# Gabrielcb/DaliID

Measured on AMD Instinct MI355X. Metric: images/sec (train step), higher is better.
Workload: dtype bf16; 1 GPU; configs[1]: ResNet-50 ReID bf16 256x128, PK batch 16x16=256 per GPU, center+proxy heads, Adam, EMA; global_batch=256, per_gpu_batch=256, parallelism=dp1

## Files before the change

daliid_amd/csrc/conv.hip:

```cpp
#include "gemm_tile.h"
#include "kernels.h"
#include <cstdlib>
#include <type_traits>
#include <vector>
#include <string>
#include <cstdio>

namespace dali {

__device__ __forceinline__ void decode_pixel(const GatherGeom& g, int p, int& n, int& ho, int& wo) {
    if (g.lhw >= 0 && g.lw >= 0) {
        n = p >> g.lhw;
        const int rem = p & ((1 << g.lhw) - 1);
        ho = rem >> g.lw;
        wo = rem & ((1 << g.lw) - 1);
    } else {
        const int hw = g.Hout * g.Wout;
        n = p / hw;
        const int rem = p - n * hw;
        ho = rem / g.Wout;
        wo = rem - ho * g.Wout;
    }
}

// ... 1370 lines not shown
    const int bn = n0 + c16 * 8;
    const bool b_ok = bn < a.Ntot;
    const int tap = b_ok ? bn / g.Ck : 0;
    const int ci = bn - tap * g.Ck;
    const int r = tap / g.S, s = tap - r * g.S;
    const int p_begin = wk.p_begin, p_end = wk.p_end, ksteps = wk.ksteps;

    auto issue = [&](int kt, int stage) {
        uint16_t* sa = smem + stage * 2 * TILE;
        uint16_t* sb = sa + TILE;
#pragma unroll
        for (int i = 0; i < 2; ++i) {
            const int blk = wave + 4 * i;
            const int p = p_begin + kt * 32 + 4 * blk + r_in;
            uint32_t oa = DMA_OOB, ob = DMA_OOB;
            if (p < p_end) {
                if (a_ok) oa = (uint32_t)(p * a.Cm + am) * 2u;
                if (b_ok) {
                    int n, ho, wo;
                    decode_pixel(g, p, n, ho, wo);
                    const int hi = ho * g.stride - g.pad + r, wi = wo * g.stride - g.pad + s;
                    if ((unsigned)hi < (unsigned)g.Hin && (unsigned)wi < (unsigned)g.Win)
                        ob = (uint32_t)((int)((long long)n * g.img_pitch) + hi * g.row_pitch + wi * g.pix_pitch + ci) * 2u;
                }
            }
            __builtin_amdgcn_raw_ptr_buffer_load_lds(rs.y, (lds_void_ptr)(sa + blk * 512), 16, oa, 0, 0, 0);
            __builtin_amdgcn_raw_ptr_buffer_load_lds(rs.x, (lds_void_ptr)(sb + blk * 512), 16, ob, 0, 0, 0);
        }
    };

    f32x4_t acc[4][4];
#pragma unroll
    for (int i = 0; i < 4; ++i)
#pragma unroll
        for (int j = 0; j < 4; ++j) acc[i][j] = f32x4_t{0.f, 0.f, 0.f, 0.f};
    const bool do_cs = COLSUM && tn == 0 && wn == 0;
    f32x4_t cs[4];
#pragma unroll
    for (int i = 0; i < 4; ++i) cs[i] = f32x4_t{0.f, 0.f, 0.f, 0.f};
    typedef short ones_vec_t __attribute__((ext_vector_type(8)));
    const bf16x8_t ones = __builtin_bit_cast(bf16x8_t, ones_vec_t{0x3F80, 0x3F80, 0x3F80, 0x3F80, 0x3F80, 0x3F80, 0x3F80, 0x3F80});

    if (ksteps > 0) {
        issue(0, 0);
        if (ksteps > 1) issue(1, 1);
        if (ksteps > 1) dma_wait<4>(); else dma_wait<0>();
        __builtin_amdgcn_s_barrier();
        conv_stamp(a, 1);
        int st_cur = 0, st_nxt2 = 2;
        for (int kt = 0; kt < ksteps; ++kt) {
            if (kt + 2 < ksteps) issue(kt + 2, st_nxt2);
            const uint16_t* sa = smem + st_cur * 2 * TILE;
            const uint16_t* sb = sa + TILE;
            bf16x8_t fa[4];
            wgrad_tr_kstep(sa, wm * 4, sb, wn * 4, lane, acc, fa);
            if constexpr (COLSUM) if (do_cs) {
#pragma unroll
                for (int i = 0; i < 4; ++i) cs[i] = __builtin_amdgcn_mfma_f32_16x16x32_bf16(fa[i], ones, cs[i], 0, 0, 0);
            }
            if (kt + 2 < ksteps) dma_wait<4>(); else dma_wait<0>();
            __builtin_amdgcn_s_barrier();
            st_cur = (st_cur == 2) ? 0 : st_cur + 1;
            st_nxt2 = (st_nxt2 == 2) ? 0 : st_nxt2 + 1;
        }
    }
    conv_stamp(a, 2);
    float* slab = a.partial + (size_t)ks * a.Cm * a.Ntot;
    store_slab_tiles<4, 4>(slab, acc, m0 + wm * 64, n0 + wn * 64, a.Cm, a.Ntot, lane);
    if constexpr (COLSUM) if (do_cs && (lane & 15) == 0) {
#pragma unroll
        for (int i = 0; i < 4; ++i)
#pragma unroll
            for (int rr = 0; rr < 4; ++rr) {
                const int m = m0 + wm * 64 + i * 16 + (lane >> 4) * 4 + rr;
                if (m < a.Cm) a.colsum[(size_t)ks * a.Cm + m] = cs[i][rr];
            }
    }
    conv_stamp_stores(a);
}

__device__ __forceinline__ int halo_swz(int row) { return ((row >> 1) & 1) | (((row >> 3) & 1) << 1); }
constexpr int W3_A_ELEMS = 32 * 128, W3_B_ELEMS = 16 * 512, W3_STAGE = W3_A_ELEMS + W3_B_ELEMS;

template <int NSTAGE>
__global__ __launch_bounds__(512) void igemm_wgrad3x3_kernel(WGradArgs a, int tiles_m, int tiles_n) {
    extern __shared__ __attribute__((aligned(16))) uint16_t smem[];
    const int tid = threadIdx.x, lane = tid & 63;
    const int wave = __builtin_amdgcn_readfirstlane(tid >> 6);
    const int wm = wave >> 2, wn = wave & 3;
    WGradWork wk;
    if (!wk.map_xcd(a, tiles_m, tiles_n)) return;
    const int ks = wk.ks, m0 = wk.tm * 128, ci0 = wk.tn * 64;
    conv_stamp(a, 0);
    const bool m_active = m0 + wm * 64 < a.Cm;
    const GatherGeom g = a.g;
    const int W = g.Wout, H = g.Hout, Cin = g.Ck, lw = g.lw, lhw = g.lhw;
    const int RW = 32 >> lw, HC = W + 2, HP = (RW + 2) * HC;
    const WGradRsrc rs = wgrad_rsrc(a);

    const int r_in = lane >> 4, ps = lane & 15;
    const int c16 = ((((ps >> 1) ^ wg_swz(4 * wave + r_in)) << 1) | (ps & 1));
    const int am = m0 + c16 * 8;
    const bool a_ok = am < a.Cm;
    int hb_hr[2], hb_off[2];
    bool hb_ok[2];
#pragma unroll
    for (int i = 0; i < 2; ++i) {
        const int hp = 8 * (wave + 8 * i) + (lane >> 3);
        const int lc = (lane & 7) ^ (halo_swz(hp) << 1);
        const int hr = hp / HC, hc = hp - hr * HC;
        hb_hr[i] = hr;
        hb_ok[i] = hp < HP && (unsigned)(hc - 1) < (unsigned)W && ci0 + lc * 8 < Cin;
        hb_off[i] = ((hc - 1) * Cin + ci0 + lc * 8) * 2;
    }
    const int p_begin = wk.p_begin, p_end = wk.p_end, ksteps = wk.ksteps;

    auto issue = [&](int kt, int stage) {
        uint16_t* sa = smem + stage * W3_STAGE;
        uint16_t* sb = sa + W3_A_ELEMS;
        const int p0 = p_begin + kt * 32;
        const int p = p0 + 4 * wave + r_in;
        const uint32_t oa = (p < p_end && a_ok) ? (uint32_t)(p * a.Cm + am) * 2u : DMA_OOB;
        __builtin_amdgcn_raw_ptr_buffer_load_lds(rs.y, (lds_void_ptr)(sa + wave * 512), 16, oa, 0, 0, 0);
        const int n = p0 >> lhw, h_base = (p0 & ((1 << lhw) - 1)) >> lw;
        const int row_bytes = W * Cin * 2;
        const int img_base = (int)((long long)n * g.img_pitch * 2);
#pragma unroll
        for (int i = 0; i < 2; ++i) {
            const int h = h_base - 1 + hb_hr[i];
            const bool ok = hb_ok[i] && (unsigned)h < (unsigned)H && p0 < p_end;
            const uint32_t ob = ok ? (uint32_t)(img_base + h * row_bytes + hb_off[i]) : DMA_OOB;
            __builtin_amdgcn_raw_ptr_buffer_load_lds(rs.x, (lds_void_ptr)(sb + (wave + 8 * i) * 512), 16, ob, 0, 0, 0);
        }
    };

    f32x4_t acc[9][4];
#pragma unroll
    for (int t = 0; t < 9; ++t)
#pragma unroll
        for (int i = 0; i < 4; ++i) acc[t][i] = f32x4_t{0.f, 0.f, 0.f, 0.f};
    const int gq = lane >> 4, q = (lane & 15) >> 2, pp = lane & 3;
    const int hrow_base = ((8 * gq) >> lw) * HC + ((8 * gq) & (W - 1)) + q;
    int boff0[9], boff1[9];
#pragma unroll
    for (int r = 0; r < 3; ++r)
#pragma unroll
        for (int s2 = 0; s2 < 3; ++s2) {
            const int row0 = hrow_base + r * HC + s2, row1 = row0 + 4;
            boff0[r * 3 + s2] = row0 * 64 + ((wn ^ halo_swz(row0)) << 4) + 4 * pp;
            boff1[r * 3 + s2] = row1 * 64 + ((wn ^ halo_swz(row1)) << 4) + 4 * pp;
        }
    auto load_b = [&](const uint16_t* sb, int t) -> TrPair { return TrPair{ds_read_tr_raw(sb + boff0[t]), ds_read_tr_raw(sb + boff1[t])}; };

    constexpr int AHEAD = NSTAGE - 1;
    auto wait_inflight = [&](int n) {
        if (n <= 0) dma_wait<0>();
        else if (n == 1) dma_wait<3>();
        else if (n == 2) dma_wait<6>();
        else if (n == 3) dma_wait<9>();
        else dma_wait<12>();
    };
    static_assert(AHEAD >= 1 && AHEAD <= 5, "ring depth");
    if (ksteps > 0) {
        int issued = 0;
        for (; issued < AHEAD && issued < ksteps; ++issued) issue(issued, issued);
        wait_inflight(issued - 1 > 4 ? 4 : issued - 1);
        __builtin_amdgcn_s_barrier();
        conv_stamp(a, 1);
        int st_cur = 0, st_fill = AHEAD % NSTAGE;
        for (int kt = 0; kt < ksteps; ++kt) {
            if (kt + AHEAD < ksteps) issue(kt + AHEAD, st_fill);
            const uint16_t* sa = smem + st_cur * W3_STAGE;
            const uint16_t* sb = sa + W3_A_ELEMS;
            if (m_active) {
            TrPair ra[4], rb[9];
#pragma unroll
            for (int i = 0; i < 4; ++i) ra[i] = tr_frag_raw(sa, wm * 4 + i, lane);
#pragma unroll
            for (int t = 0; t < 9; ++t) rb[t] = load_b(sb, t);
            tr_settle<18>(ra[0], ra[1], ra[2], ra[3]);
            tr_settle<10>(rb[0], rb[1], rb[2], rb[3]);
            bf16x8_t fa[4];
#pragma unroll
            for (int i = 0; i < 4; ++i) fa[i] = tr_join(ra[i]);
#pragma unroll
            for (int t = 0; t < 4; ++t) {
                const bf16x8_t fb = tr_join(rb[t]);
#pragma unroll
                for (int i = 0; i < 4; ++i) acc[t][i] = __builtin_amdgcn_mfma_f32_16x16x32_bf16(fa[i], fb, acc[t][i], 0, 0, 0);
            }
            __builtin_amdgcn_sched_barrier(0);
            tr_settle<0>(rb[4], rb[5], rb[6], rb[7]);
            tr_settle_all(rb[8]);
#pragma unroll
            for (int t = 4; t < 9; ++t) {
                const bf16x8_t fb = tr_join(rb[t]);
#pragma unroll
                for (int i = 0; i < 4; ++i) acc[t][i] = __builtin_amdgcn_mfma_f32_16x16x32_bf16(fa[i], fb, acc[t][i], 0, 0, 0);
            }
            }
            const int left = ksteps - 1 - kt;
            const int keep = (left < AHEAD ? left : AHEAD) - 1;
            wait_inflight(keep > 4 ? 4 : keep);
            __builtin_amdgcn_s_barrier();
            st_cur = (st_cur == NSTAGE - 1) ? 0 : st_cur + 1;
            st_fill = (st_fill == NSTAGE - 1) ? 0 : st_fill + 1;
        }
    }
    conv_stamp(a, 2);
    float* slab = a.partial + (size_t)ks * a.Cm * a.Ntot;
    if (m_active) {
        float* row = slab + (size_t)(m0 + wm * 64 + (lane >> 4) * 4) * a.Ntot + ci0 + wn * 16 + (lane & 15);
#pragma unroll
        for (int i = 0; i < 4; ++i)
#pragma unroll
            for (int rr = 0; rr < 4; ++rr) {
                float* p = row + (size_t)(i * 16 + rr) * a.Ntot;
#pragma unroll
                for (int t = 0; t < 9; ++t) p[t * Cin] = acc[t][i][rr];
            }
    }
    conv_stamp_stores(a);
}

template <int WM, int WN, int NSTAGE, bool COLSUM = false>
__global__ __launch_bounds__(WM * WN * 64, 4) void igemm_wgrad_wg_kernel(WGradArgs a, int tiles_m, int tiles_n) {
    constexpr int TM = 64 * WM, TN = 64 * WN, NW = WM * WN;
    using Gather = WGradGather<TM / 128, (TM + TN) / 128, NW>;
    constexpr int IMG = Gather::IMG, NIMG_A = Gather::NIMG_A, STAGE = Gather::STAGE, NDMA = Gather::NDMA;
    constexpr int AHEAD = NSTAGE - 1;
    static_assert(TM % 128 == 0 && TN % 128 == 0, "unsupported wave grid");
    extern __shared__ __attribute__((aligned(16))) uint16_t smem[];
    const int tid = threadIdx.x, lane = tid & 63;
    const int wave = __builtin_amdgcn_readfirstlane(tid >> 6);
    const int wm = wave / WN, wn = wave % WN;
    WGradWork wk;
    if (!wk.map_xcd(a, tiles_m, tiles_n)) return;
    const int m0 = wk.tm * TM, n0 = wk.tn * TN, ksteps = wk.ksteps;
    const Gather gather(a, wave, m0, n0, wk.p_begin, wk.p_end, lane);

    const bool do_cs = COLSUM && wn == 0;
    int cs_turn = wk.tn;
    f32x4_t cs = f32x4_t{0.f, 0.f, 0.f, 0.f};
    typedef unsigned sel_vec_t __attribute__((ext_vector_type(4)));
    const int cs_col = (lane & 15) >> 2;
    f32x4_t acc[4][4];
// ... 351 lines not shown

int gemm_profile_begin(hipStream_t st, int cls, double flops, const char* what) {
    if (!g_prof || g_prof->used >= g_prof->cap) return -1;
    const size_t i = g_prof->used++;
    g_prof->cls[i] = cls; g_prof->flops[i] = flops; g_prof->desc[i] = what;
    (void)hipEventRecord(g_prof->ev[2 * i], st);
    return (int)i;
}
void gemm_profile_end(hipStream_t st, int slot) {
    if (slot >= 0 && g_prof) (void)hipEventRecord(g_prof->ev[2 * slot + 1], st);
}

enum GemmGrid {
    GRID_XCD,
    GRID_CLASSES,
    GRID_CUS,
    GRID_HALO,
    GRID_SPLITS,
    GRID_SPLITS8,
};
struct GemmKernel {
    const void* fn;
    int block;
    int lds;
    int tm, tn;
    GemmGrid grid;
    int plan_wgs = 0;
    int f1_rb = 0;
    mutable DeviceOnce once{};
};
template <class F> static const void* kfn(F* f) { return reinterpret_cast<const void*>(f); }
constexpr int ring_lds(int tm, int tn, int k_tile, int stages) { return (tm + tn) * k_tile * 2 * stages; }
constexpr int REG128_LDS = GemmCfg<128, 128, 1, 1, 1>::LDS_BYTES, REG64_LDS = GemmCfg<64, 256, 1, 1, 1>::LDS_BYTES;
constexpr int DMA128_LDS = REG128_LDS / 2 * 3, DMA64_LDS = REG64_LDS / 2 * 3;
constexpr int HALO64_LDS = (3 * 64 * 64 + HALO64_PX * 64) * 2;

static const GemmKernel
    CONV128_BN{kfn(&igemm_conv_kernel<128, 128, true>), 256, REG128_LDS, 128, 128, GRID_XCD},
    CONV128{kfn(&igemm_conv_kernel<128, 128, false>), 256, REG128_LDS, 128, 128, GRID_XCD},
    DMA128{kfn(&igemm_conv_dma_kernel<128, 128, 3>), 256, DMA128_LDS, 128, 128, GRID_XCD},
    DMA128_LIN{kfn(&igemm_conv_dma_kernel<128, 128, 3, Epi::LIN>), 256, DMA128_LDS, 128, 128, GRID_XCD},
    DMA128_FUSED{kfn(&igemm_conv_dma_kernel<128, 128, 3, Epi::FUSED>), 256, DMA128_LDS, 128, 128, GRID_XCD},
    DMA128_CLS{kfn(&igemm_conv_dma_kernel<128, 128, 3, Epi::PARITY>), 256, DMA128_LDS, 128, 128, GRID_CLASSES},
    DMA128_SRC2{kfn(&igemm_conv_dma_kernel<128, 128, 3, Epi::CONV, true>), 256, DMA128_LDS, 128, 128, GRID_XCD},
    CONV64_BN{kfn(&igemm_conv_kernel<64, 256, true>), 256, REG64_LDS, 64, 256, GRID_XCD},
    CONV64{kfn(&igemm_conv_kernel<64, 256, false>), 256, REG64_LDS, 64, 256, GRID_XCD},
    DMA64{kfn(&igemm_conv_dma_kernel<64, 256, 3>), 256, DMA64_LDS, 64, 256, GRID_XCD},
    DMA64_LEAN{kfn(&igemm_conv_dma_kernel<64, 256, 3, Epi::FUSED_LEAN>), 256, DMA64_LDS, 64, 256, GRID_XCD},
    DMA64_SRC2{kfn(&igemm_conv_dma_kernel<64, 256, 3, Epi::CONV, true>), 256, DMA64_LDS, 64, 256, GRID_XCD},
    K64S64{kfn(&igemm_conv_k64s_kernel<1, 4, 4, 2>), 512, ring_lds(64, 256, 64, 2), 64, 256, GRID_XCD},
    HALO64{kfn(&igemm_conv_halo64_kernel<3>), 512, HALO64_LDS, 64, 256, GRID_HALO},
    HALO64_LEAN{kfn(&igemm_conv_halo64_kernel<3, Epi::FUSED_LEAN>), 512, HALO64_LDS, 64, 256, GRID_HALO},
    WG128{kfn(&igemm_conv_wg_kernel<2, 4, 3>), 512, ring_lds(128, 256, 32, 3), 128, 256, GRID_XCD},
    WG128_LIN{kfn(&igemm_conv_wg_kernel<2, 4, 3, Epi::LIN>), 512, ring_lds(128, 256, 32, 3), 128, 256, GRID_XCD},
    WG128_FUSED{kfn(&igemm_conv_wg_kernel<2, 4, 3, Epi::FUSED>), 512, ring_lds(128, 256, 32, 3), 128, 256, GRID_XCD},
    WG128_CLS{kfn(&igemm_conv_wg_kernel<2, 4, 3, Epi::PARITY>), 512, ring_lds(128, 256, 32, 3), 128, 256, GRID_CLASSES},
    WG256{kfn(&igemm_conv_wg_kernel<4, 4, 4>), 1024, ring_lds(256, 256, 32, 4), 256, 256, GRID_XCD},
    K64S{kfn(&igemm_conv_k64s_kernel<2, 4, 8, 3>), 1024, ring_lds(128, 256, 64, 3), 128, 256, GRID_XCD},
    K64S_LIN{kfn(&igemm_conv_k64s_kernel<2, 4, 8, 3, 4, 4, Epi::LIN>), 1024, ring_lds(128, 256, 64, 3), 128, 256, GRID_XCD},
    K64S_LEAN{kfn(&igemm_conv_k64s_kernel<2, 4, 8, 3, 4, 4, Epi::FUSED_LEAN>), 1024, ring_lds(128, 256, 64, 3), 128, 256, GRID_XCD},
    K64S_SRC2{kfn(&igemm_conv_k64s_kernel<2, 4, 8, 3, 4, 4, Epi::CONV, true>), 1024, ring_lds(128, 256, 64, 3), 128, 256, GRID_XCD},
    K64{kfn(&igemm_conv_k64_kernel<4, 4, 2>), 1024, ring_lds(256, 256, 64, 2), 256, 256, GRID_XCD},
    K64_LIN{kfn(&igemm_conv_k64_kernel<4, 4, 2, 4, 4, Epi::LIN>), 1024, ring_lds(256, 256, 64, 2), 256, 256, GRID_XCD},
    K64_FUSED{kfn(&igemm_conv_k64_kernel<4, 4, 2, 4, 4, Epi::FUSED>), 1024, ring_lds(256, 256, 64, 2), 256, 256, GRID_XCD},
    K64_CLS{kfn(&igemm_conv_k64_kernel<4, 4, 2, 4, 4, Epi::PARITY>), 1024, ring_lds(256, 256, 64, 2), 256, 256, GRID_CLASSES},
    K64_SRC2{kfn(&igemm_conv_k64_kernel<4, 4, 2, 4, 4, Epi::CONV, true>), 1024, ring_lds(256, 256, 64, 2), 256, 256, GRID_XCD},
    K64_FUSED_SRC2{kfn(&igemm_conv_k64_kernel<4, 4, 2, 4, 4, Epi::FUSED, true>), 1024, ring_lds(256, 256, 64, 2), 256, 256, GRID_XCD},
    K64_320{kfn(&igemm_conv_k64_kernel<4, 4, 2, 4, 5, Epi::LIN>), 1024, ring_lds(256, 320, 64, 2), 256, 320, GRID_XCD};

template <int RB, bool RES, bool OM, bool BITS, bool SRC2 = false>
static GemmKernel f1_kernel() {
    return {kfn(&fused1x1_persist_kernel<3, RB, RES, OM, BITS, SRC2>), (F1_NC + F1_NP + F1_NR) * 64, f1_lds_bytes(3, RB, RB == 2 ? 128 : F1_KMAX),
            F1_TM, F1_TN, GRID_CUS, 0, RB};
}
static const GemmKernel F1[2][2][2][2] = {
    {{{f1_kernel<2, false, false, false, true>(), f1_kernel<2, false, false, true>()}, {f1_kernel<2, false, true, false>(), f1_kernel<2, false, true, true>()}},
     {{f1_kernel<2, true, false, false>(), f1_kernel<2, true, false, true>()}, {f1_kernel<2, true, true, false>(), f1_kernel<2, true, true, true>()}}},
    {{{f1_kernel<1, false, false, false, true>(), f1_kernel<1, false, false, true>()}, {f1_kernel<1, false, true, false>(), f1_kernel<1, false, true, true>()}},
     {{f1_kernel<1, true, false, false>(), f1_kernel<1, true, false, true>()}, {f1_kernel<1, true, true, false>(), f1_kernel<1, true, true, true>()}}}};

static const GemmKernel
    WG_BN{kfn(&igemm_wgrad_kernel<true>), 256, 0, 128, 128, GRID_SPLITS},
    WG_PLAIN{kfn(&igemm_wgrad_kernel<false>), 256, 0, 128, 128, GRID_SPLITS},
    WG_3X3{kfn(&igemm_wgrad3x3_kernel<3>), 512, 3 * W3_STAGE * 2, 128, 9 * 64, GRID_SPLITS8, 256};
static const GemmKernel WG_DMA[2] = {
    {kfn(&igemm_wgrad_dma_kernel<false>), 256, 0, 128, 128, GRID_SPLITS8},
    {kfn(&igemm_wgrad_dma_kernel<true>), 256, 0, 128, 128, GRID_SPLITS8}};
static const GemmKernel WG_WG[2] = {
    {kfn(&igemm_wgrad_wg_kernel<2, 4, 3>), 512, ring_lds(128, 256, 32, 3), 128, 256, GRID_SPLITS8, 512},
    {kfn(&igemm_wgrad_wg_kernel<2, 4, 3, true>), 512, ring_lds(128, 256, 32, 3), 128, 256, GRID_SPLITS8, 512}};
static const GemmKernel WG_P[2][2] = {
    {{kfn(&igemm_wgrad_p_kernel<2, 4, 4, 4, 8, 6>), 1024, ring_lds(128, 256, 32, 6), 128, 256, GRID_SPLITS8, 256},
     {kfn(&igemm_wgrad_p_kernel<2, 4, 4, 4, 8, 6, true>), 1024, ring_lds(128, 256, 32, 6), 128, 256, GRID_SPLITS8, 256}},
    {{kfn(&igemm_wgrad_p_kernel<1, 4, 8, 4, 4, 6>), 512, ring_lds(128, 256, 32, 6), 128, 256, GRID_SPLITS8, 256},
     {kfn(&igemm_wgrad_p_kernel<1, 4, 8, 4, 4, 6, true>), 512, ring_lds(128, 256, 32, 6), 128, 256, GRID_SPLITS8, 256}}};

struct GemmChoice {
    const GemmKernel* k = nullptr;
    int tiles_m = 0, tiles_n = 0, lds = 0, class_grid = 0;
    unsigned grid = 0;
    int rc = DALI_OK, why_arg = 0;
    const char* why = nullptr;
    GemmChoice() = default;
    GemmChoice(int rc_, const char* why_, int why_arg_ = 0) : rc(rc_), why_arg(why_arg_), why(why_) {}
    int refuse() const { set_error(why, why_arg); return rc; }
};
static GemmChoice gemm_place(const GemmKernel& k, int rows, int cols, int mult, int Ck) {
    GemmChoice c;
    c.k = &k;
    c.tiles_m = (rows + k.tm - 1) / k.tm;
    c.tiles_n = (cols + k.tn - 1) / k.tn;
    c.lds = k.f1_rb ? f1_lds_bytes(3, k.f1_rb, Ck) : k.lds;
    switch (k.grid) {
        case GRID_XCD: c.grid = xcd_tile_grid(c.tiles_m, c.tiles_n); break;
        case GRID_CLASSES: c.class_grid = xcd_tile_grid(c.tiles_m, c.tiles_n); c.grid = mult * c.class_grid; break;
        case GRID_CUS: c.grid = mult; break;
        case GRID_HALO: c.grid = c.tiles_n; break;
        case GRID_SPLITS: c.grid = c.tiles_m * c.tiles_n * mult; break;
        case GRID_SPLITS8: c.grid = (c.tiles_m * c.tiles_n * mult + 7) / 8 * 8; break;
    }
    return c;
}
template <class Args>
static int gemm_launch(hipStream_t st, const GemmChoice& c, Args& args) {
    const GemmKernel& k = *c.k;
    DeviceOnce::Guard once(k.once);
    if (k.lds > 64 * 1024 && once.first()) {
        DALI_HIP(hipFuncSetAttribute(k.fn, hipFuncAttributeMaxDynamicSharedMemorySize, k.lds));
        once.done();
    }
    int tiles_m = c.tiles_m, tiles_n = c.tiles_n;
    void* tile_args[] = {&args, &tiles_m, &tiles_n};
    void* halo_args[] = {&args, &tiles_n};
    (void)hipLaunchKernel(k.fn, dim3(c.grid), dim3(k.block), k.grid == GRID_HALO ? halo_args : tile_args, c.lds, st);
    DALI_LAUNCH_CHECK();
    return DALI_OK;
}

static unsigned long long* g_conv_stamps = nullptr;

static bool dma_addressable(long long bytes) { return bytes < 0x7ff00000ll; }
static bool gather_dma_ok(const GatherGeom& g, int P, long long other_bytes) {
    return dma_addressable(g.img_pitch * 2 * ((P + g.Hout * g.Wout - 1) / (g.Hout * g.Wout))) && dma_addressable(other_bytes);
}
static bool conv_dma_ok(const IGemmArgs& a) { return !a.in_scale && gather_dma_ok(a.g, a.P, (long long)a.Cm * a.g.R * a.g.S * a.g.Ck * 2); }
static bool plain_rows(const GatherGeom& g) {
    return g.R == 1 && g.S == 1 && g.stride == 1 && g.pad == 0 && g.pix_pitch == g.Ck && g.row_pitch == g.Win * g.Ck &&
           g.img_pitch == (long long)g.Hin * g.Win * g.Ck && g.Hin == g.Hout && g.Win == g.Wout;
}
static bool halo64_ok(const IGemmArgs& a) {
    const GatherGeom& g = a.g;
    return a.Cm == 64 && g.Ck == 64 && g.R == 3 && g.S == 3 && g.stride == 1 && g.pad == 1 && !g.sub && (g.Wout == 16 || g.Wout == 32) &&
           ilog2_exact(g.Hout * g.Wout) >= 8 && g.Hin == g.Hout && g.Win == g.Wout && g.pix_pitch == 64 && g.row_pitch == g.Win * 64 &&
           g.img_pitch == (long long)g.Hin * g.Win * 64 && a.P % 256 == 0;
}

static int f1_cu_count() {
    static int n_cus = 0;
    if (!n_cus) {
        int dev = 0, v = 0;
        if (hipGetDevice(&dev) != hipSuccess || hipDeviceGetAttribute(&v, hipDeviceAttributeMultiprocessorCount, dev) != hipSuccess) { set_error("conv: device query failed"); return -1; }
        n_cus = v > 8 ? v & ~7 : 8;
    }
    return n_cus;
}
static bool f1_fills(int Cm, int P, int n_cus) {
    const int tiles_m = Cm / F1_TM, tiles_n = (P + F1_TN - 1) / F1_TN;
// ... 65 lines not shown
    if (k64 && cfg == CONV_256x256) return use(a.X2 ? K64_SRC2 : lin ? K64_LIN : K64);
    if (k64 && cfg == CONV_128x256) return use(a.X2 ? K64S_SRC2 : lin ? K64S_LIN : K64S);
    if (narrow_k64 && !lin && halo64_ok(a)) return use(HALO64);
    if (narrow_k64) return use(K64S64);
    if (narrow) return use(in_bn ? CONV64_BN : !dma_ok ? CONV64 : a.X2 ? DMA64_SRC2 : DMA64);
    if (dma_ok && cfg == CONV_256x256) return use(WG256);
    if (dma_ok && cfg == CONV_128x256) return use(lin ? WG128_LIN : WG128);
    return use(in_bn ? CONV128_BN : !dma_ok ? CONV128 : a.X2 ? DMA128_SRC2 : lin ? DMA128_LIN : DMA128);
}

static int launch_igemm_conv_one(hipStream_t st, const IGemmArgs& a) {
    IGemmArgs args = a;
    args.g.lw = ilog2_exact(a.g.Wout);
    args.g.lhw = ilog2_exact(a.g.Hout * a.g.Wout);
    const GemmChoice c = conv_choose(args, f1_cu_count());
    if (c.rc == DALI_ERR_LIMIT) return c.refuse();
    const int K = a.g.nr * a.g.ns * a.g.Ck;
    char what[160] = "";
    if (g_prof)
        snprintf(what, sizeof what, "%s,Cm=%d,K=%d,P=%d,taps=%d,stride=%d,sub=%d,fused=%d,stats=%d,res=%d,mask=%d,lin=%d", a.g.mode ? "dgrad" : "fwd", a.Cm, K, a.P,
                 a.g.R * a.g.S, a.g.stride, a.g.sub, a.out_scale ? 1 : 0, a.stats ? 1 : 0, a.Res ? 1 : 0, (a.res_mask || a.out_mask) ? 1 : 0,
                 (a.bias || a.row_scale || a.act) ? 1 : 0);
    ProfScope prof_scope(st, 0, a.g.sub == 2 ? 2.0 * a.Cm * (double)a.P * a.g.R * a.g.S * a.g.Ck : 2.0 * a.Cm * (double)a.P * K, what);
    if (!c.k) return c.refuse();
    const int stat_tiles = a.stats ? igemm_conv_stat_tiles(a.Cm, a.P, K, a.in_scale != nullptr) : c.tiles_n;
    if (stat_tiles != c.tiles_n) {
        set_error("conv: the statistics slab has %d pixel tiles, the chosen kernel %d", stat_tiles, c.tiles_n);
        return DALI_ERR_UNSUPPORTED;
    }
    if (c.k->grid == GRID_CLASSES) args.g.class_grid = c.class_grid;
    return gemm_launch(st, c, args);
}

int launch_igemm_conv(hipStream_t st, const IGemmArgs& a) {
    IGemmArgs args = a;
    args.stamps = g_conv_stamps;
    GatherGeom& g = args.g;
    g.sub = 0; g.oph = g.opw = 0; g.Hfull = g.Hout; g.Wfull = g.Wout;
    g.r0 = 0; g.rstep = 1; g.nr = g.R; g.s0 = 0; g.sstep = 1; g.ns = g.S;
    if (g.mode == 1 && g.stride == 2 && conv_dma_ok(args) && !a.stats && (g.Hout % 2) == 0 && (g.Wout % 2) == 0 &&
        ilog2_exact(g.Wout / 2) >= 0 && ilog2_exact((g.Hout / 2) * (g.Wout / 2)) >= 0) {
        int nr[2], ns[2];
        for (int ph = 0; ph < 2; ++ph) {
            const int r0 = (ph + g.pad) & 1, s0 = (ph + g.pad) & 1;
            nr[ph] = r0 < g.R ? (g.R - r0 + 1) / 2 : 0;
            ns[ph] = s0 < g.S ? (g.S - s0 + 1) / 2 : 0;
        }
        const bool all_have = nr[0] && nr[1] && ns[0] && ns[1];
        if (all_have && a.Cm > 64 && (a.Cm & 7) == 0) {
            IGemmArgs s = args;
            s.g.sub = 2; s.g.oph = s.g.opw = 0; s.g.Hfull = g.Hout; s.g.Wfull = g.Wout;
            s.g.Hout = g.Hout / 2; s.g.Wout = g.Wout / 2; s.P = a.P / 4;
            s.g.r0 = s.g.s0 = 0; s.g.rstep = s.g.sstep = 2;
            s.g.nr = nr[0] > nr[1] ? nr[0] : nr[1]; s.g.ns = ns[0] > ns[1] ? ns[0] : ns[1];
            return launch_igemm_conv_one(st, s);
        }
        if (all_have || (a.Res != nullptr && a.Res == a.O)) {
            for (int ph = 0; ph < 2; ++ph)
                for (int pw = 0; pw < 2; ++pw) {
                    if (nr[ph] * ns[pw] == 0) continue;
                    IGemmArgs s = args;
                    s.g.sub = 1; s.g.oph = ph; s.g.opw = pw; s.g.Hfull = g.Hout; s.g.Wfull = g.Wout;
                    s.g.Hout = g.Hout / 2; s.g.Wout = g.Wout / 2; s.P = a.P / 4;
                    s.g.r0 = (ph + g.pad) & 1; s.g.rstep = 2; s.g.nr = nr[ph];
                    s.g.s0 = (pw + g.pad) & 1; s.g.sstep = 2; s.g.ns = ns[pw];
                    const int rc = launch_igemm_conv_one(st, s);
                    if (rc) return rc;
                }
            return DALI_OK;
        }
    }
    return launch_igemm_conv_one(st, args);
}

static bool wgrad_spec(int Cm, int Ntot) { return ((Cm + 127) / 128) * ((Ntot + 255) / 256) <= 100; }
int wgrad_pick_cfg(int Cm, int Ntot, int taps, int P, int halo_w) {
    if (taps == 9 && (halo_w == 8 || halo_w == 16 || halo_w == 32) && Cm % 64 == 0 && (Ntot / 9) % 64 == 0 && P % 32 == 0) return 3;
    if (taps == 7 && Ntot == 224 && P >= 16384) return 2;
    return (taps == 1 && Ntot >= 256 && P >= 16384) ? 2 : 0;
}
static const GemmKernel& wgrad_kernel(int cfg, int Cm, int Ntot, bool in_bn, bool dma_ok, bool colsum, bool flat) {
    if (in_bn) return WG_BN;
    if (!dma_ok) return WG_PLAIN;
    if (cfg == 3) return WG_3X3;
    if (cfg == 2) return wgrad_spec(Cm, Ntot) ? WG_P[flat][colsum] : WG_WG[colsum];
    return WG_DMA[colsum];
}
static bool wgrad_colsum_ok(int cfg, bool in_bn, bool dma_ok) { return cfg != 3 && !in_bn && dma_ok; }
static int colsum_rows_of(const GemmKernel& k, int Ntot, int splits) { return k.tn == 128 ? splits : splits * ((Ntot + k.tn - 1) / k.tn); }

void wgrad_plan(int Cm, int Ntot, int P, int target_blocks, int* splits, int* pix_per_split, size_t* ws_bytes, int taps, int halo_w) {
    const GemmKernel& k = wgrad_kernel(wgrad_pick_cfg(Cm, Ntot, taps, P, halo_w), Cm, Ntot, false, true, false, true);
    if (k.plan_wgs) target_blocks = k.plan_wgs;
    const int tiles = ((Cm + k.tm - 1) / k.tm) * ((Ntot + k.tn - 1) / k.tn);
    int sp = (target_blocks + tiles - 1) / tiles;
    const int max_sp = (P + 255) / 256;
    if (sp > max_sp) sp = max_sp;
    if (sp < 1) sp = 1;
    {
        int best = sp;
        double best_cost = (double)((tiles * sp + target_blocks - 1) / target_blocks) / sp;
        for (int c = sp - 1; c >= 1 && c >= sp / 2; --c) {
            const double cost = (double)((tiles * c + target_blocks - 1) / target_blocks) / c;
            if (cost <= best_cost + 1e-12) { best = c; best_cost = cost; }
        }
        sp = best;
    }
    int pps = ((P + sp - 1) / sp + 31) & ~31;
    sp = (P + pps - 1) / pps;
    *splits = sp; *pix_per_split = pps;
    *ws_bytes = (size_t)sp * Cm * Ntot * sizeof(float);
}

static GemmChoice wgrad_choose(const WGradArgs& a) {
    const GatherGeom& g = a.g;
    const bool dma_ok = gather_dma_ok(g, a.P, (long long)a.P * a.Cm * 2);
    const bool halo = g.R == 3 && g.S == 3 && g.stride == 1 && g.pad == 1 && g.mode == 0 && g.lw >= 0 && g.lhw >= 7 && g.Hin == g.Hout && g.Win == g.Wout &&
                      g.pix_pitch == g.Ck && g.row_pitch == g.Win * g.Ck;
    const int cfg = wgrad_pick_cfg(a.Cm, a.Ntot, g.R * g.S, a.P, halo ? g.Wout : 0);
    if (a.colsum && !wgrad_colsum_ok(cfg, a.in_scale != nullptr, dma_ok))
        return GemmChoice(DALI_ERR_INVALID, "wgrad: column sums ride on the 128 x 128 and 128 x 256 LDS-DMA kernels only (wgrad_colsum_supported)");
    return gemm_place(wgrad_kernel(cfg, a.Cm, a.Ntot, a.in_scale != nullptr, dma_ok, a.colsum != nullptr, plain_rows(g)), a.Cm, a.Ntot, a.splits, g.Ck);
}

int launch_igemm_wgrad(hipStream_t st, const WGradArgs& a, float* out, int accumulate, float* colsum_out, int colsum_rows) {
    WGradArgs args = a;
    args.stamps = g_conv_stamps;
    args.g.lw = ilog2_exact(a.g.Wout);
    args.g.lhw = ilog2_exact(a.g.Hout * a.g.Wout);
    const GemmChoice c = wgrad_choose(args);
    {
    char what[160] = "";
    if (g_prof)
        snprintf(what, sizeof what, "wgrad,Cm=%d,K=%d,P=%d,taps=%d,stride=%d,sub=0,fused=%d,stats=0,res=0,mask=0,lin=%d", a.Cm, a.Ntot, a.P, a.g.R * a.g.S, a.g.stride,
                 a.in_scale ? 1 : 0, a.colsum ? 1 : 0);
    ProfScope prof_scope(st, 1, 2.0 * a.Cm * (double)a.Ntot * a.P, what);
    if (!c.k) return c.refuse();
    if (a.colsum && colsum_out && colsum_rows != colsum_rows_of(*c.k, a.Ntot, a.splits)) {
        set_error("wgrad: %d column-sum rows passed, the chosen kernel leaves %d", colsum_rows, colsum_rows_of(*c.k, a.Ntot, a.splits));
        return DALI_ERR_UNSUPPORTED;
    }
    if (int rc = gemm_launch(st, c, args)) return rc;
    }
    if (!out) return DALI_OK;
    return launch_splitk_reduce2(st, a.partial, out, (size_t)a.Cm * a.Ntot, a.splits, accumulate, (a.colsum && colsum_out) ? a.colsum : nullptr, colsum_out,
                                 (size_t)a.Cm, colsum_rows);
}

int wgrad_colsum_rows(int Cm, int Ntot, int taps, int P, int splits) {
    return colsum_rows_of(wgrad_kernel(wgrad_pick_cfg(Cm, Ntot, taps, P, 0), Cm, Ntot, false, true, true, true), Ntot, splits);
}
bool wgrad_colsum_supported(int Cm, int Ntot, int taps, int P) {
    return wgrad_colsum_ok(wgrad_pick_cfg(Cm, Ntot, taps, P, 0), false, dma_addressable((long long)P * Cm * 2) && dma_addressable((long long)P * Ntot * 2));
}

int launch_splitk_reduce(hipStream_t st, const float* partial, float* out, size_t elems, int splits, int accumulate) {
    return launch_splitk_reduce2(st, partial, out, elems, splits, accumulate, nullptr, nullptr, 0, 0);
}
int launch_splitk_reduce2(hipStream_t st, const float* partial, float* out, size_t elems, int splits, int accumulate,
                          const float* partial2, float* out2, size_t elems2, int splits2) {
    const size_t chunks = (elems + 3) / 4;
    const unsigned rblocks = (unsigned)((chunks + 63) / 64);
    const int W = splits >= 32 ? 16 : (splits >= 2 ? 4 : 1);
    const bool second = partial2 && out2 && elems2 > 0;
    if (second && ((elems & 3) || (elems2 & 3))) {
        if (int rc = launch_splitk_reduce2(st, partial, out, elems, splits, accumulate, nullptr, nullptr, 0, 0)) return rc;
        return launch_splitk_reduce2(st, partial2, out2, elems2, splits2, 0, nullptr, nullptr, 0, 0);
    }
    if (elems & 3) {
        hipLaunchKernelGGL(splitk_reduce_odd_kernel, dim3((unsigned)((elems + 255) / 256)), dim3(256), 0, st, partial, out, elems, splits, accumulate, W);
        DALI_LAUNCH_CHECK();
        return DALI_OK;
    }
    ReduceJob2 j2{nullptr, nullptr, 0, 0, 0xffffffffu};
    unsigned grid = rblocks;
    if (second) { j2 = ReduceJob2{partial2, out2, elems2, splits2, rblocks}; grid += (unsigned)((elems2 / 4 + 63) / 64); }
    switch (W) {
        case 1: hipLaunchKernelGGL(splitk_reduce_kernel<1>, dim3(grid), dim3(64), 0, st, partial, out, elems, splits, accumulate, j2); break;
        case 4: hipLaunchKernelGGL(splitk_reduce_kernel<4>, dim3(grid), dim3(256), 0, st, partial, out, elems, splits, accumulate, j2); break;
        default: hipLaunchKernelGGL(splitk_reduce_kernel<16>, dim3(grid), dim3(1024), 0, st, partial, out, elems, splits, accumulate, j2); break;
    }
    DALI_LAUNCH_CHECK();
    return DALI_OK;
}

}

extern "C" int dali_debug_set_conv_stamps(void* dev_ptr) { g_conv_stamps = static_cast<unsigned long long*>(dev_ptr); return DALI_OK; }
extern "C" int dali_debug_wgrad_splits(int Cm, int Ntot, int P, int taps, int halo_w) {
    int sp = 0, pps = 0; size_t wsb = 0;
    wgrad_plan(Cm, Ntot, P, 512, &sp, &pps, &wsb, taps, halo_w);
    return sp;
}
extern "C" int dali_debug_splitk_reduce(void* stream, const float* partial, float* out, long long elems, int splits, int accumulate) {
    return launch_splitk_reduce(static_cast<hipStream_t>(stream), partial, out, (size_t)elems, splits, accumulate);
}

extern "C" int dali_gemm_profile_begin(dali_ctx* ctx, int max_launches) {
    DALI_REQUIRE(ctx && max_launches > 0, "dali_gemm_profile_begin: bad argument");
    DALI_REQUIRE(!g_prof, "dali_gemm_profile_begin: a profile is already open");
    GemmProfiler* p = new GemmProfiler();
    p->cap = (size_t)max_launches;
    p->ev.resize(2 * p->cap); p->cls.resize(p->cap); p->flops.resize(p->cap); p->desc.resize(p->cap);
    for (auto& e : p->ev) DALI_HIP(hipEventCreate(&e));
    g_prof = p;
    return DALI_OK;
}

extern "C" int dali_gemm_profile_end(dali_ctx* ctx, double* total_ms, double* total_flops, long long* launches) {
    DALI_REQUIRE(ctx && total_ms && total_flops && launches, "dali_gemm_profile_end: null argument");
    DALI_REQUIRE(g_prof, "dali_gemm_profile_end: no open profile");
    GemmProfiler* p = g_prof;
    g_prof = nullptr;
    for (int c = 0; c < 2; ++c) { total_ms[c] = 0; total_flops[c] = 0; launches[c] = 0; }
    int rc = DALI_OK;
    const char* dump_path = getenv("DALI_GEMM_PROFILE_DUMP");
    FILE* dump = dump_path ? fopen(dump_path, "a") : nullptr;
    for (size_t i = 0; i < p->used; ++i) {
        float ms = 0.f;
        if (hipEventSynchronize(p->ev[2 * i + 1]) != hipSuccess || hipEventElapsedTime(&ms, p->ev[2 * i], p->ev[2 * i + 1]) != hipSuccess) {
            set_error("gemm_profile_end: event query failed"); rc = DALI_ERR_HIP; break;
        }
        total_ms[p->cls[i]] += ms; total_flops[p->cls[i]] += p->flops[i]; launches[p->cls[i]] += 1;
        if (dump) fprintf(dump, "%zu,%s,us=%.2f,gflop=%.3f\n", i, p->desc[i].c_str(), ms * 1e3, p->flops[i] * 1e-9);
    }
    if (dump) fclose(dump);
    for (auto& e : p->ev) (void)hipEventDestroy(e);
    delete p;
    return rc;
}

static int fill_geom(GatherGeom& g, int n_img, int Hin, int Win, int Ck, int Hout, int Wout, int R, int S, int stride, int pad, int mode) {
    g.Hout = Hout; g.Wout = Wout; g.Hin = Hin; g.Win = Win; g.Ck = Ck; g.R = R; g.S = S; g.stride = stride; g.pad = pad;
    g.mode = mode;
    g.pix_pitch = Ck; g.row_pitch = Win * Ck; g.img_pitch = (long long)Hin * Win * Ck;
    g.lw = g.lhw = -1;
    (void)n_img;
    return 0;
}

extern "C" int dali_conv2d_fwd(dali_ctx* ctx, void* stream, const uint16_t* x, const uint16_t* w, uint16_t* y,
                               int n, int h, int wd, int cin, int cout, int r, int s, int stride, int pad,
                               const float* in_scale, const float* in_shift, int in_relu, float* stats) {
    DALI_REQUIRE(ctx && x && w && y, "dali_conv2d_fwd: null argument");
    DALI_REQUIRE(cin % 32 == 0 && cout % 4 == 0, "dali_conv2d_fwd: cin must be a multiple of 32 and cout of 4 (cin=%d cout=%d)", cin, cout);
    DALI_REQUIRE(stride == 1 || stride == 2, "dali_conv2d_fwd: stride %d unsupported", stride);
    DALI_REQUIRE((in_scale == nullptr) == (in_shift == nullptr), "dali_conv2d_fwd: in_scale/in_shift must come together");
    const int ho = (h + 2 * pad - r) / stride + 1, wo = (wd + 2 * pad - s) / stride + 1;
    IGemmArgs a{};
    a.W = w; a.X = x; a.O = y; a.Res = nullptr; a.in_scale = in_scale; a.in_shift = in_shift; a.stats = stats;
    a.Cm = cout; a.P = n * ho * wo; a.in_relu = in_relu;
    fill_geom(a.g, n, h, wd, cin, ho, wo, r, s, stride, pad, 0);
    return launch_igemm_conv((hipStream_t)stream, a);
}

extern "C" int dali_conv2d_bn_act(dali_ctx* ctx, void* stream, const uint16_t* x, const uint16_t* w, uint16_t* y, int n, int h, int wd, int cin, int cout,
                                  int r, int s, int stride, int pad, const float* out_scale, const float* out_shift, int out_relu) {
    DALI_REQUIRE(ctx && x && w && y && out_scale && out_shift, "dali_conv2d_bn_act: null argument");
    DALI_REQUIRE(cin % 32 == 0 && cout % 8 == 0, "dali_conv2d_bn_act: cin must be a multiple of 32 and cout of 8 (cin=%d cout=%d)", cin, cout);
    DALI_REQUIRE(stride == 1 || stride == 2, "dali_conv2d_bn_act: stride %d unsupported", stride);
    const int ho = (h + 2 * pad - r) / stride + 1, wo = (wd + 2 * pad - s) / stride + 1;
    IGemmArgs a{};
    a.W = w; a.X = x; a.O = y;
    a.out_scale = out_scale; a.out_shift = out_shift; a.out_relu = out_relu;
    a.Cm = cout; a.P = n * ho * wo;
    fill_geom(a.g, n, h, wd, cin, ho, wo, r, s, stride, pad, 0);
    return launch_igemm_conv((hipStream_t)stream, a);
}

static int halo_width(int r, int s, int stride, int pad, int ho, int wo) {
    return (r == 3 && s == 3 && stride == 1 && pad == 1 && ilog2_exact(wo) >= 0 && ilog2_exact(ho * wo) >= 0 && ho * wo >= 128) ? wo : 0;
}
extern "C" int dali_conv2d_stat_tiles(int cout, int cin, int r, int s, int stride, int pad, int n, int ho, int wo, int fused_operand) {
    (void)stride; (void)pad;
    return igemm_conv_stat_tiles(cout, n * ho * wo, r * s * cin, fused_operand != 0);
// ... 145 lines not shown
```

include/daliid_debug.h:

```cpp
#ifndef DALIID_DEBUG_H
#define DALIID_DEBUG_H

#ifdef __cplusplus
extern "C" {
#endif

int dali_debug_reload_env(void);

int dali_debug_set_conv_stamps(void* dev_ptr);

int dali_debug_wgrad_splits(int Cm, int Ntot, int P, int taps, int halo_w);

int dali_debug_splitk_reduce(void* stream, const float* partial, float* out, long long elems, int splits, int accumulate);

struct dali_resnet;
int dali_debug_resnet_backward_block(struct dali_resnet* net, void* stream, const float* d_emb, int block);

#ifdef __cplusplus
}
#endif
#endif
```

Baseline: 17810 images/s.

## Split k-steps across wave halves in 3x3 wgrad kernel when Cm is 64

Adds a KPAIR variant of the 3x3 weight-gradient kernel for layers with Cm<=64. In the existing kernel the upper-M waves have no work for these layers. In the new variant the two wave rows each process alternate k-steps from a deeper six-stage ring. Their accumulators are then summed through LDS at the end. This aims to use the otherwise idle waves in layer1's 64-channel 3x3 convs, at the cost of twice the LDS footprint and an extra LDS reduction.

```diff
diff --git a/daliid_amd/csrc/conv.hip b/daliid_amd/csrc/conv.hip
--- a/daliid_amd/csrc/conv.hip
+++ b/daliid_amd/csrc/conv.hip
@@ -1476,7 +1476,7 @@
 __device__ __forceinline__ int halo_swz(int row) { return ((row >> 1) & 1) | (((row >> 3) & 1) << 1); }
 constexpr int W3_A_ELEMS = 32 * 128, W3_B_ELEMS = 16 * 512, W3_STAGE = W3_A_ELEMS + W3_B_ELEMS;
 
-template <int NSTAGE>
+template <int NSTAGE, bool KPAIR = false>
 __global__ __launch_bounds__(512) void igemm_wgrad3x3_kernel(WGradArgs a, int tiles_m, int tiles_n) {
     extern __shared__ __attribute__((aligned(16))) uint16_t smem[];
     const int tid = threadIdx.x, lane = tid & 63;
@@ -1555,7 +1555,77 @@
         else dma_wait<12>();
     };
     static_assert(AHEAD >= 1 && AHEAD <= 5, "ring depth");
-    if (ksteps > 0) {
+    if constexpr (KPAIR) {
+        constexpr int NSLOT = NSTAGE / 2, AHEAD2 = NSLOT - 1;
+        static_assert(NSTAGE % 2 == 0 && AHEAD2 >= 1 && AHEAD2 <= 2, "ring depth in k-step pairs");
+        static_assert(NSTAGE * W3_STAGE * 2 >= 4 * 36 * 64 * 16, "the ring holds the upper half's accumulators");
+        auto issue2 = [&](int it, int slot) { issue(2 * it, 2 * slot); issue(2 * it + 1, 2 * slot + 1); };
+        auto wait_inflight2 = [&](int n) {
+            if (n <= 0) dma_wait<0>();
+            else if (n == 1) dma_wait<6>();
+            else dma_wait<12>();
+        };
+        const int iters = (ksteps + 1) >> 1;
+        if (iters > 0) {
+            int issued = 0;
+            for (; issued < AHEAD2 && issued < iters; ++issued) issue2(issued, issued);
+            wait_inflight2(issued - 1);
+            __builtin_amdgcn_s_barrier();
+            conv_stamp(a, 1);
+            int sl_cur = 0, sl_fill = AHEAD2 % NSLOT;
+            for (int it = 0; it < iters; ++it) {
+                if (it + AHEAD2 < iters) issue2(it + AHEAD2, sl_fill);
+                if (2 * it + wm < ksteps) {
+                    const uint16_t* sa = smem + (2 * sl_cur + wm) * W3_STAGE;
+                    const uint16_t* sb = sa + W3_A_ELEMS;
+                    TrPair ra[4], rb[9];
+#pragma unroll
+                    for (int i = 0; i < 4; ++i) ra[i] = tr_frag_raw(sa, i, lane);
+#pragma unroll
+                    for (int t = 0; t < 9; ++t) rb[t] = load_b(sb, t);
+                    tr_settle<18>(ra[0], ra[1], ra[2], ra[3]);
+                    tr_settle<10>(rb[0], rb[1], rb[2], rb[3]);
+                    bf16x8_t fa[4];
+#pragma unroll
+                    for (int i = 0; i < 4; ++i) fa[i] = tr_join(ra[i]);
+#pragma unroll
+                    for (int t = 0; t < 4; ++t) {
+                        const bf16x8_t fb = tr_join(rb[t]);
+#pragma unroll
+                        for (int i = 0; i < 4; ++i) acc[t][i] = __builtin_amdgcn_mfma_f32_16x16x32_bf16(fa[i], fb, acc[t][i], 0, 0, 0);
+                    }
+                    __builtin_amdgcn_sched_barrier(0);
+                    tr_settle<0>(rb[4], rb[5], rb[6], rb[7]);
+                    tr_settle_all(rb[8]);
+#pragma unroll
+                    for (int t = 4; t < 9; ++t) {
+                        const bf16x8_t fb = tr_join(rb[t]);
+#pragma unroll
+                        for (int i = 0; i < 4; ++i) acc[t][i] = __builtin_amdgcn_mfma_f32_16x16x32_bf16(fa[i], fb, acc[t][i], 0, 0, 0);
+                    }
+                }
+                const int left = iters - 1 - it;
+                wait_inflight2((left < AHEAD2 ? left : AHEAD2) - 1);
+                __builtin_amdgcn_s_barrier();
+                sl_cur = (sl_cur == NSLOT - 1) ? 0 : sl_cur + 1;
+                sl_fill = (sl_fill == NSLOT - 1) ? 0 : sl_fill + 1;
+            }
+        }
+        f32x4_t* xch = reinterpret_cast<f32x4_t*>(smem) + (size_t)wn * 36 * 64 + lane;
+        if (wm == 1) {
+#pragma unroll
+            for (int t = 0; t < 9; ++t)
+#pragma unroll
+                for (int i = 0; i < 4; ++i) xch[(t * 4 + i) * 64] = acc[t][i];
+        }
+        lds_barrier();
+        if (wm == 0) {
+#pragma unroll
+            for (int t = 0; t < 9; ++t)
+#pragma unroll
+                for (int i = 0; i < 4; ++i) acc[t][i] = acc[t][i] + xch[(t * 4 + i) * 64];
+        }
+    } else if (ksteps > 0) {
         int issued = 0;
         for (; issued < AHEAD && issued < ksteps; ++issued) issue(issued, issued);
         wait_inflight(issued - 1 > 4 ? 4 : issued - 1);
@@ -2073,7 +2143,8 @@
 static const GemmKernel
     WG_BN{kfn(&igemm_wgrad_kernel<true>), 256, 0, 128, 128, GRID_SPLITS},
     WG_PLAIN{kfn(&igemm_wgrad_kernel<false>), 256, 0, 128, 128, GRID_SPLITS},
-    WG_3X3{kfn(&igemm_wgrad3x3_kernel<3>), 512, 3 * W3_STAGE * 2, 128, 9 * 64, GRID_SPLITS8, 256};
+    WG_3X3{kfn(&igemm_wgrad3x3_kernel<3>), 512, 3 * W3_STAGE * 2, 128, 9 * 64, GRID_SPLITS8, 256},
+    WG_3X3_C64{kfn(&igemm_wgrad3x3_kernel<6, true>), 512, 6 * W3_STAGE * 2, 128, 9 * 64, GRID_SPLITS8, 256};
 static const GemmKernel WG_DMA[2] = {
     {kfn(&igemm_wgrad_dma_kernel<false>), 256, 0, 128, 128, GRID_SPLITS8},
     {kfn(&igemm_wgrad_dma_kernel<true>), 256, 0, 128, 128, GRID_SPLITS8}};
@@ -2305,7 +2376,7 @@
 static const GemmKernel& wgrad_kernel(int cfg, int Cm, int Ntot, bool in_bn, bool dma_ok, bool colsum, bool flat) {
     if (in_bn) return WG_BN;
     if (!dma_ok) return WG_PLAIN;
-    if (cfg == 3) return WG_3X3;
+    if (cfg == 3) return Cm <= 64 ? WG_3X3_C64 : WG_3X3;
     if (cfg == 2) return wgrad_spec(Cm, Ntot) ? WG_P[flat][colsum] : WG_WG[colsum];
     return WG_DMA[colsum];
 }
@@ -2414,6 +2485,9 @@
     int sp = 0, pps = 0; size_t wsb = 0;
     wgrad_plan(Cm, Ntot, P, 512, &sp, &pps, &wsb, taps, halo_w);
     return sp;
+}
+extern "C" int dali_debug_wgrad_is_3x3_c64(int Cm, int Ntot, int P, int taps, int halo_w) {
+    return &wgrad_kernel(wgrad_pick_cfg(Cm, Ntot, taps, P, halo_w), Cm, Ntot, false, true, false, true) == &WG_3X3_C64;
 }
 extern "C" int dali_debug_splitk_reduce(void* stream, const float* partial, float* out, long long elems, int splits, int accumulate) {
     return launch_splitk_reduce(static_cast<hipStream_t>(stream), partial, out, (size_t)elems, splits, accumulate);
diff --git a/include/daliid_debug.h b/include/daliid_debug.h
--- a/include/daliid_debug.h
+++ b/include/daliid_debug.h
@@ -10,6 +10,7 @@
 int dali_debug_set_conv_stamps(void* dev_ptr);
 
 int dali_debug_wgrad_splits(int Cm, int Ntot, int P, int taps, int halo_w);
+int dali_debug_wgrad_is_3x3_c64(int Cm, int Ntot, int P, int taps, int halo_w);
 
 int dali_debug_splitk_reduce(void* stream, const float* partial, float* out, long long elems, int splits, int accumulate);
 
```

Result: no change. 17730 images/s (-0.5%).
